# xiezhy6/PASTA-GAN-plusplus

Measured on AMD Instinct MI355X. Metric: 512-res try-on images/sec (SynthesisNetwork fwd), higher is better.
Workload: dtype f32

## Files before the change

### include/pasta_gan_ops.h

```cpp
#ifndef PASTA_GAN_OPS_H
#define PASTA_GAN_OPS_H

#include <stdint.h>

#ifdef __cplusplus
extern "C" {
#endif

#define PG_ABI_VERSION 20

enum pg_dtype { PG_F32 = 0, PG_F16 = 1, PG_BF16 = 2, PG_F64 = 3 };

enum pg_error {
    PG_OK = 0,
    PG_ERR_INVALID_ARG = -1,
    PG_ERR_UNSUPPORTED = -2,
    PG_ERR_TOO_LARGE = -3
};

enum pg_act {
    PG_ACT_LINEAR = 1, PG_ACT_RELU = 2, PG_ACT_LRELU = 3, PG_ACT_TANH = 4, PG_ACT_SIGMOID = 5,
    PG_ACT_ELU = 6, PG_ACT_SELU = 7, PG_ACT_SOFTPLUS = 8, PG_ACT_SWISH = 9
};

int pg_bias_act(const void* x, const void* b, const void* xref, const void* yref, const void* dy, void* y,
                int dtype, int64_t sizeX, int sizeB, int64_t stepB,
                int grad, int act, float alpha, float gain, float clamp, void* stream);
int pg_bias_act_abi_version(void);

int64_t pg_bias_act_grad_bias_workspace(int dtype, int64_t sizeX, int sizeB, int64_t stepB);
int pg_bias_act_grad_bias(const void* dy, const void* yref, void* dx, void* db, void* workspace, int64_t workspace_bytes,
                          int dtype, int64_t sizeX, int sizeB, int64_t stepB,
                          int act, float alpha, float gain, float clamp, void* stream);

int pg_upfirdn2d(const void* x, const float* f, void* y, int dtype,
                 int N, int C, int inH, int inW, const int64_t xstride[4],
                 int fh, int fw, const int64_t fstride[2],
                 int outH, int outW, const int64_t ystride[4],
                 int upx, int upy, int downx, int downy, int padx0, int pady0,
                 int flip, float gain, void* stream);
int pg_upfirdn2d_with_odd_samples(const void* x, const float* f, void* y, float* y_odd, int dtype,
                                  int N, int C, int inH, int inW, const int64_t xstride[4],
// ... 83 lines not shown
    const float* w2[PG_MODCONV_PREP_MAX_JOBS];
    const float* styles[PG_MODCONV_PREP_MAX_JOBS];
    float*       out[PG_MODCONV_PREP_MAX_JOBS];
    float*       s_norm[PG_MODCONV_PREP_MAX_JOBS];
    void*        s16[PG_MODCONV_PREP_MAX_JOBS];
    int          cout[PG_MODCONV_PREP_MAX_JOBS];
    int          cin[PG_MODCONV_PREP_MAX_JOBS];
    int          flags[PG_MODCONV_PREP_MAX_JOBS];
    int          njobs;
    int          half_dtype;
} pg_modconv_prep_jobs;
int pg_modconv_prep_batched(const pg_modconv_prep_jobs* jobs, int N, void* stream);

int pg_conv2d_up2_forward(const float* x, const float* packed, float* y, int N, int Cin, int H, int W, int Cout,
                          const int64_t ystride[4], const float* in_scale, const float* out_scale, void* stream);
int pg_conv2d_up2_splitk_plan(int N, int Cin, int H, int W, int Cout);
int pg_conv2d_up2_forward_splitk(const float* x, const float* packed, float* y, int N, int Cin, int H, int W, int Cout,
                                 const int64_t ystride[4], const float* in_scale, const float* out_scale, float* workspace, int ksplit, void* stream);

int64_t pg_conv2d_up2x3_packed_size(int Cout, int Cin);
int pg_conv2d_up2x3_pack_weight(const float* packed, void* packed_x3, int Cout, int Cin, void* stream);
int pg_conv2d_up2x3_forward(const float* x, const float* packed, const void* packed_x3, float* y, int N, int Cin, int H, int W, int Cout,
                            const int64_t ystride[4], const float* in_scale, const float* out_scale, float* edge_column, void* stream);

int64_t pg_conv2d_stem7x3_packed_size(int Cout);
int pg_conv2d_stem7x3_pack_weight(const float* w, void* packed, int Cout, float scale, int flip_hw, void* stream);
int pg_conv2d_stem7x3_forward(const float* x, const void* packed, float* y, int N, int H, int W, int Cout, const int64_t ystride[4],
                              const pg_conv2d_fusion* fusion, void* stream);

int64_t pg_conv2d_s2x3_packed_size(int Cout, int Cin);
int pg_conv2d_s2x3_pack_weight(const float* packed, void* packed_x3, int Cout, int Cin, void* stream);
int pg_conv2d_s2x3_forward(const float* x, const void* packed_x3, float* y, int N, int Cin, int H, int W, int Cout, const int64_t ystride[4],
                           const pg_conv2d_fusion* fusion, void* stream);

int pg_conv1x1_small(const float* x, const float* w, const float* styles, const float* bias, const float* skip, float* y,
                     int N, int Cin, int64_t HW, int Cout, float scale, float clamp, void* stream);

int pg_conv1x1_fold_prep(const float* wm, const float* bm, const float* wh, const float* bh, const float* styles, float* w_out, float* b_out,
                         int N, int Cm, int C, int Cout, void* stream);
int pg_conv1x1_fold_heads(const float* x, const float* x2, const float* w, const float* bias, const float* skip, float* y_a, float* y_b,
                          int N, int C1, int C2, int64_t HW, int Cout, int c_a, int n_skip, float clamp, void* stream);

int pg_conv3x3_fold_head(const float* xa, const float* xb, const float* w, const float* bias, const float* skip, float* y,
                         int N, int C, int H, int W, int Cout, float clamp, void* stream);

int pg_conv3x3_cin1(const float* x, const float* w, float* y, int N, int H, int W, int Cout, float scale, int act, void* stream);

int pg_instance_norm_stats(const float* x, float* mean, float* rstd, int NC, int64_t HW, float eps, void* stream);
int pg_spade_norm(const float* x, const float* mean, const float* rstd, const float* gamma, const float* beta,
                  float* y, int NC, int64_t HW, void* stream);

#define PG_STATS16_MAX_CHUNKS 256
int pg_instance_norm_stats_cl16(const void* x, float* mean, float* rstd, float* workspace, int dtype, int N, int64_t HW, int C, float eps, void* stream);
int pg_spade_combine_cl16(const void* x, const float* mean, const float* rstd, const void* gamma_beta, void* y, int dtype, int N, int64_t HW, int C,
                          int act, float alpha, float gain, float clamp, void* stream);

int pg_spade_train_forward(const float* x, const float* mean, const float* rstd, const float* gamma, const float* beta, float* y,
                           int N, int C, int64_t HW, int64_t gamma_sample_stride, int64_t beta_sample_stride, void* stream);
int pg_spade_train_backward(const float* dy, const float* x, const float* mean, const float* rstd, const float* gamma, float* sums,
                            float* dx, float* dgamma, float* dbeta, int N, int C, int64_t HW,
                            int64_t gamma_sample_stride, int64_t dgamma_sample_stride, int64_t dbeta_sample_stride, void* stream);

int pg_spade_masked_sums(const float* feat, const float* mask, const float* denorm_mask, float* sums, float* counts,
                         int N, int C, int H, int W, void* stream);
int pg_spade_feat_assemble(const float* feat_upper, const float* feat_lower, const float* mask_upper, const float* mask_lower,
                           const float* denorm_mask_upper, const float* denorm_mask_lower,
// ... 251 lines not shown
```

### pasta-gan-plusplus_amd/torch_utils/custom_ops.py

```python

import concurrent.futures
import ctypes
import fcntl
import glob
import hashlib
import os
import re
import shutil
import subprocess
import sys

verbosity = 'brief'

CSRC_DIR = os.path.normpath(os.path.join(os.path.dirname(os.path.abspath(__file__)), '..', 'csrc'))
INCLUDE_DIR = os.path.normpath(os.path.join(CSRC_DIR, '..', '..', 'include'))
DEV_DIR = os.path.join(CSRC_DIR, 'dev')
OFFLOAD_ARCH = 'gfx950'
HIPCC_FLAGS = ['-O3', '-std=c++17', '-fPIC', '-fvisibility=hidden', f'--offload-arch={OFFLOAD_ARCH}']

PLUGIN_SOURCES = {
    'bias_act_plugin': ['bias_act.hip'],
    'upfirdn2d_plugin': ['upfirdn2d.hip'],
    'patch_routing_plugin': ['patch_routing.hip'],
    'augment_plugin': ['augment.hip'],
    'tryon_plugin': ['tryon.hip'],
    'tryon_front_plugin': ['tryon_front.hip'],
    'train_fetch_plugin': ['train_fetch.hip'],
    'snapshot_grid_plugin': ['snapshot_grid.hip'],
    'vgg_loss_plugin': ['vgg_loss.hip'],
    'image_metrics_plugin': ['image_metrics.hip'],
    'conv2d_plugin': ['conv2d.hip', 'conv2d_inst_k3s1.hip', 'conv2d_inst_k1s1.hip', 'conv2d_inst_k2x2.hip', 'conv2d_inst_k2x1.hip',
                      'conv2d_inst_k1x2.hip', 'conv2d_inst_k7s1.hip', 'conv2d_inst_k3s2.hip', 'conv2d_inst_k1s2.hip', 'conv2d_inst_wino.hip', 'conv2d_inst_wino4.hip', 'conv2d_inst_wino4s.hip', 'conv2d_inst_wino4t.hip', 'conv2d_inst_wino4x.hip', 'conv2d_inst_wino4xs.hip', 'conv2d_inst_wino4xt.hip', 'conv2d_inst_wino4b.hip', 'conv2d_inst_wino4bs.hip', 'conv2d_inst_up2.hip', 'conv2d_inst_stem7.hip', 'conv2d_inst_s2x3.hip', 'conv2d_inst_s1x1.hip',
                      'conv2d_wgrad.hip', 'conv2d16.hip', 'conv2d16_inst_k3s1.hip', 'conv2d16_inst_k3s1b.hip', 'conv2d16_inst_k1s1.hip', 'conv2d16_inst_k2x2.hip', 'conv2d16_inst_k2x1.hip',
                      'conv2d16_inst_k1x2.hip', 'conv2d16_inst_k3s2.hip', 'conv2d16_inst_up2f.hip', 'conv1x1_head16.hip', 'spade16.hip', 'conv1x1_fold.hip', 'conv3x3_fold.hip', 'optim.hip'],
}

ABI_VERSION = 20

_cached_plugins = dict()


class NativePlugin:

    def __init__(self, name, path, abi_name=None):
        self.name = name
        self.path = path
        self.lib = ctypes.CDLL(path)
        probe = getattr(self.lib, 'pg_' + (abi_name or name).replace('_plugin', '') + '_abi_version', None)
        if probe is None:
            raise RuntimeError(f'{path} does not export its ABI version; rebuild it from csrc/')
        probe.restype = ctypes.c_int
        if probe() != ABI_VERSION:
            raise RuntimeError(f'{path} implements ABI version {probe()}, the bindings expect {ABI_VERSION}; rebuild it from csrc/')

    def __repr__(self):
        return f'<NativePlugin {self.name} at {self.path}>'


def _find_hipcc():
    for cand in (os.environ.get('HIPCC'), shutil.which('hipcc'), '/opt/rocm/bin/hipcc'):
        if cand and os.path.isfile(cand):
            return cand
    return None


def _digest(sources, extra_flags):
    h = hashlib.md5()
    deps = sorted(set(list(sources) + glob.glob(os.path.join(CSRC_DIR, '*.h')) + glob.glob(os.path.join(INCLUDE_DIR, '*.h'))))
    for path in deps:
        h.update(os.path.basename(path).encode())
# ... 180 lines not shown
```

### pasta-gan-plusplus_amd/torch_utils/ops/conv2d_gradfix.py

```python

import contextlib
import os

import weakref

import torch

from . import _native as nat
from . import bias_act
from . import conv2d_mfma
from . import conv2d_mfma16

native_input_gradients = os.environ.get('PG_NATIVE_DGRAD', '1') == '1'
native_weight_gradients16 = os.environ.get('PG_NATIVE_WGRAD16', '1') == '1'
native_weight_gradients = os.environ.get('PG_NATIVE_WGRAD', '1') == '1'
enabled = True
weight_gradients_disabled = False


@contextlib.contextmanager
def no_weight_gradients():
    global weight_gradients_disabled
    old = weight_gradients_disabled
    weight_gradients_disabled = True
# ... 117 lines not shown
    if hit is None:
        w = weight.detach()
        if not w.is_contiguous():
            w = w.contiguous()
        hit = conv2d_mfma.pack_weight(w, flip=flip, transpose_oi=transpose_oi, winograd=winograd)
        if sum(e[1].numel() * e[1].element_size() for e in _pack_cache.values()) + hit.numel() * hit.element_size() > _PACK_CACHE_MAX_BYTES:
            _pack_cache.clear()

        def _evict(ref, key=key):
            e = _pack_cache.get(key)
            if e is not None and e[0] is ref:
                del _pack_cache[key]
        _pack_cache[key] = (weakref.ref(base, _evict), hit)
    return hit


def _epilogue_backward(ctx, dy, y, ep, want_b):
    act, alpha, gain, clamp = ep
    if want_b:
        return bias_act._BiasActGrad.apply(dy, None, None, y, 1, act, alpha, gain, clamp, True)
    return bias_act._BiasActGrad.apply(dy, None, None, y, 1, act, alpha, gain, clamp), None


class _Conv2dMfma(torch.autograd.Function):
    @staticmethod
    def forward(ctx, x, weight, bias, stride, padding, transposed, output_padding, ep=None):
        x = x.contiguous()
        n, cin, h, w = x.shape
        kh, kw = int(weight.shape[2]), int(weight.shape[3])
        if not transposed:
            cout = int(weight.shape[0])
            fz = dict(act=ep[0], alpha=ep[1], gain=ep[2], clamp=ep[3] if ep[3] >= 0 else None) if ep is not None else {}
            wg = conv2d_mfma.use_winograd(kh, kw, stride, cout, cin, pad=padding, hw=(h, w), ep=fz)
            y = conv2d_mfma.conv2d_forward(x, _packed(weight, wg), cout, kh, kw, stride=stride, pad=padding, bias=bias, winograd=wg, s2x3=False, **fz)
        else:
            assert ep is None
            cout = int(weight.shape[1])
            out_hw = ((h - 1) * stride - 2 * padding[0] + kh + output_padding[0], (w - 1) * stride - 2 * padding[1] + kw + output_padding[1])
            if ((kh, kw, stride) == (3, 3, 2) and tuple(padding) == (0, 0) and tuple(output_padding) == (0, 0) and bias is None and UP2_TRANSPOSED
                    and (n * cout * out_hw[0] * ((out_hw[1] + 3) // 4 * 4)) * 4 < 2 ** 31):
                main = _packed(weight, 0, flip=False, transpose_oi=True)
                packs = dict(main=main)
                if UP2_TRANSPOSED_X3 and cin % 16 == 0 and cin >= 32:
                    hit = _x3_of_pack.get(id(main))
                    if hit is None or hit[0]() is not main:
                        x3 = conv2d_mfma.pack_s2x3_planes(main, cout, cin)
                        _x3_of_pack[id(main)] = hit = (weakref.ref(main, lambda r, k=id(main): _x3_of_pack.pop(k, None)), x3)
                    packs['x3'] = hit[1]
                y = conv2d_mfma.conv_up2_forward(x, packs, cout, x3=None if 'x3' in packs else False)
            else:
                phases = conv2d_mfma.pack_transposed(weight, stride, padding, (h, w), out_hw)
                y = conv2d_mfma.conv_transpose2d_forward(x, phases, cout, out_hw, stride=stride, bias=bias)
        ctx.save_for_backward(x, weight, y if ep is not None else None)
        ctx.cfg = (stride, padding, transposed, output_padding, bias is not None, ep)
        return y

    @staticmethod
    def backward(ctx, dy):
        x, weight, y = ctx.saved_tensors
        stride, padding, transposed, output_padding, has_bias, ep = ctx.cfg
        kh, kw = int(weight.shape[2]), int(weight.shape[3])
        dx = dw = db = None
        if ep is not None:
            dy, db = _epilogue_backward(ctx, dy, y, ep, has_bias and ctx.needs_input_grad[2])
        if ctx.needs_input_grad[0] and native_input_gradients:
            dx = _input_gradient(dy, x.shape, weight, stride, padding, transposed, output_padding)
        want_w = ctx.needs_input_grad[1] and not weight_gradients_disabled
# ... 92 lines not shown
            if not transposed:
                g = conv2d_mfma16.weight_gradient(x, dy, weight.shape, padding, stride=stride)
            else:
                g = conv2d_mfma16.weight_gradient(dy, x, weight.shape, padding, stride=stride)
            dw = g.to(weight.dtype) if g is not None else None
        if want_b and db is None and (dw is not None or not want_w):
            db = bias_act.channel_sum(dy, 1)
        need_x = dx is None and ctx.needs_input_grad[0]
        need_w = want_w and dw is None
        need_b = want_b and db is None
        if need_x or need_w or need_b:
            gx, gw, gb = torch.ops.aten.convolution_backward(
                dy, x, weight.to(x.dtype), [weight.shape[1 if transposed else 0]] if has_bias else None,
                [stride, stride], list(padding), [1, 1], transposed, list(output_padding), 1, [need_x, need_w, need_b])
            dx = gx if need_x else dx
            dw = gw.to(weight.dtype) if need_w else dw
            db = gb if need_b else db
        return dx, dw, db, None, None, None, None, None


def _input_gradient(dy, x_shape, weight, stride, padding, transposed, output_padding, fn=None, mod=None):
    _Conv2dMfma, conv2d_mfma = (fn or globals()['_Conv2dMfma']), (mod or globals()['conv2d_mfma'])
    kh, kw = int(weight.shape[2]), int(weight.shape[3])
    _, _, h, w = x_shape
    if not transposed:
        if stride == 1:
            py, px = kh - 1 - padding[0], kw - 1 - padding[1]
            if min(py, px) < 0 or not conv2d_mfma.supported(kh, kw, 1):
                return None
            if fn is None and not (torch.is_grad_enabled() and (dy.requires_grad or weight.requires_grad)):
                cin_f = int(weight.shape[1])
                wg = globals()['conv2d_mfma'].use_winograd(kh, kw, 1, cin_f, int(weight.shape[0]), pad=(py, px), hw=dy.shape[2:])
                pk = _packed(weight, wg, flip=True, transpose_oi=True)
                return globals()['conv2d_mfma'].conv2d_forward(dy.contiguous(), pk, cin_f, kh, kw, stride=1, pad=(py, px), winograd=wg)
            return _Conv2dMfma.apply(dy, weight.transpose(0, 1).flip([2, 3]), None, 1, (py, px), False, (0, 0))
        opad = (h - ((dy.shape[2] - 1) * stride - 2 * padding[0] + kh), w - ((dy.shape[3] - 1) * stride - 2 * padding[1] + kw))
        if min(opad) < 0 or max(opad) >= stride or kh < stride or kw < stride:
            return None
        if not all(conv2d_mfma.supported(-(-(kh - a) // stride), -(-(kw - b) // stride), 1) for a in range(stride) for b in range(stride)):
            return None
        return _Conv2dMfma.apply(dy, weight, None, stride, padding, True, opad)
    if not conv2d_mfma.supported(kh, kw, stride) or min(padding) < 0:
        return None
    dx = _Conv2dMfma.apply(dy, weight, None, stride, padding, False, (0, 0))
    return dx if dx.shape[2:] == tuple(x_shape[2:]) else None
```

### pasta-gan-plusplus_amd/torch_utils/ops/conv2d_mfma.py

```python

import contextlib
import ctypes
import os
import weakref

import torch

from .. import custom_ops
from . import _native as nat

ACT_INDEX = {'linear': 1, 'relu': 2, 'lrelu': 3, 'tanh': 4, 'sigmoid': 5, 'elu': 6, 'selu': 7, 'softplus': 8, 'swish': 9}

FUSED_ACTS = ('linear', 'relu', 'lrelu')

SUPPORTED = {(3, 3, 1), (1, 1, 1), (2, 2, 1), (2, 1, 1), (1, 2, 1), (7, 7, 1), (3, 3, 2), (1, 1, 2)}


class Fusion(ctypes.Structure):
    _fields_ = [
        ('in_scale', ctypes.c_void_p), ('in_bias', ctypes.c_void_p), ('in_act', ctypes.c_int), ('in_alpha', ctypes.c_float),
        ('in_gain', ctypes.c_float), ('in_clamp', ctypes.c_float),
        ('out_scale', ctypes.c_void_p), ('noise', ctypes.c_void_p), ('noise_batch_stride', ctypes.c_int64), ('noise_gain', ctypes.c_float),
        ('bias', ctypes.c_void_p), ('act', ctypes.c_int), ('alpha', ctypes.c_float), ('gain', ctypes.c_float), ('clamp', ctypes.c_float),
        ('residual', ctypes.c_void_p),
# ... 90 lines not shown
        lib.pg_conv2d_wgrad_plan.argtypes = [i] * 8
        lib.pg_conv2d_wgrad.restype = i
        lib.pg_conv2d_wgrad.argtypes = [vp, vp, vp, vp] + [i] * 13 + [vp]
        lib.pg_conv2d_up2_forward.restype = i
        lib.pg_conv2d_up2_forward.argtypes = [vp, vp, vp, i, i, i, i, i, ctypes.POINTER(ctypes.c_int64), vp, vp, vp]
        lib.pg_split3_bf16_cl.restype = i
        lib.pg_split3_bf16_cl.argtypes = [vp, vp, i, i, i64, vp]
        lib.pg_conv2d16_wgrad_x3.restype = i
        lib.pg_conv2d16_wgrad_x3.argtypes = [vp, vp, vp, vp] + [i] * 13 + [vp]
        lib.pg_conv2d16_wgrad_plan.restype = i
        lib.pg_conv2d16_wgrad_plan.argtypes = [i] * 8
        lib.pg_conv2d_up2_splitk_plan.restype = i
        lib.pg_conv2d_up2_splitk_plan.argtypes = [i, i, i, i, i]
        lib.pg_conv2d_up2x3_packed_size.restype = i64
        lib.pg_conv2d_up2x3_packed_size.argtypes = [i, i]
        lib.pg_conv2d_up2x3_pack_weight.restype = i
        lib.pg_conv2d_up2x3_pack_weight.argtypes = [vp, vp, i, i, vp]
        lib.pg_conv2d_up2x3_forward.restype = i
        lib.pg_conv2d_up2x3_forward.argtypes = [vp, vp, vp, vp, i, i, i, i, i, ctypes.POINTER(ctypes.c_int64), vp, vp, vp, vp]
        lib.pg_conv2d_up2_forward_splitk.restype = i
        lib.pg_conv2d_up2_forward_splitk.argtypes = [vp, vp, vp, i, i, i, i, i, ctypes.POINTER(ctypes.c_int64), vp, vp, vp, i, vp]
        lib.pg_conv2d_stem7x3_packed_size.restype = i64
        lib.pg_conv2d_stem7x3_packed_size.argtypes = [i]
        lib.pg_conv2d_stem7x3_pack_weight.restype = i
        lib.pg_conv2d_stem7x3_pack_weight.argtypes = [vp, vp, i, ctypes.c_float, i, vp]
        lib.pg_conv2d_stem7x3_forward.restype = i
        lib.pg_conv2d_stem7x3_forward.argtypes = [vp, vp, vp, i, i, i, i, ctypes.POINTER(ctypes.c_int64), ctypes.POINTER(Fusion), vp]
        lib.pg_conv2d_s2x3_packed_size.restype = i64
        lib.pg_conv2d_s2x3_packed_size.argtypes = [i, i]
        lib.pg_conv2d_s2x3_pack_weight.restype = i
        lib.pg_conv2d_s2x3_pack_weight.argtypes = [vp, vp, i, i, vp]
        lib.pg_conv2d_s2x3_forward.restype = i
        lib.pg_conv2d_s2x3_forward.argtypes = [vp, vp, vp, i, i, i, i, i, ctypes.POINTER(i64), ctypes.POINTER(Fusion), vp]
        lib.pg_conv3x3_cin1.restype = i
        lib.pg_conv3x3_cin1.argtypes = [vp, vp, vp, i, i, i, i, f, i, vp]
        lib.pg_conv1x1_small.restype = i
        lib.pg_conv1x1_small.argtypes = [vp] * 6 + [i, i, i64, i, f, f, vp]
        lib.pg_conv1x1_fold_prep.restype = i
        lib.pg_conv1x1_fold_prep.argtypes = [vp] * 7 + [i, i, i, i, vp]
        lib.pg_conv1x1_fold_heads.restype = i
        lib.pg_conv1x1_fold_heads.argtypes = [vp] * 7 + [i, i, i, i64, i, i, i, f, vp]
        lib.pg_conv3x3_fold_head.restype = i
        lib.pg_conv3x3_fold_head.argtypes = [vp] * 6 + [i, i, i, i, i, f, vp]
        _plugin = plugin
    return _plugin


WINO_F2, WINO_F4, WINO_F4B, WINO_F4X3 = 1, 2, 3, 4
WINO_FORMS = {0: ('direct', False, False), WINO_F2: ('winograd', False, False), WINO_F4: ('winograd4', True, False),
              WINO_F4B: ('winograd4', False, True), WINO_F4X3: ('winograd4x3', True, False)}


def _wino_form(winograd):
    if int(winograd) not in WINO_FORMS:
        raise nat.NativeOpError(f'conv2d_mfma: winograd={winograd!r} is not one of the forms {sorted(WINO_FORMS)}')
    return (int(winograd), *WINO_FORMS[int(winograd)])


_WINO4B = os.environ.get('PG_WINO4B', '1')
F4_FORM = WINO_F4 if _WINO4B == '0' else WINO_F4B
F4_WIDE = WINO_F4 if os.environ.get('PG_WINO4_X3', '1') == '0' else WINO_F4X3


def f4_form(hw):
    if _WINO4B == '2':
        return WINO_F4B
# ... 68 lines not shown
        with torch.cuda.device(w.device):
            st = lib.pg_conv2d_winograd_pack_weight(form, nat.ptr(w), nat.ptr(packed), cout, cin, float(scale), int(bool(flip)), int(bool(transpose_oi)), nat.stream_of(w))
        nat.check(st, 'pg_conv2d_winograd_pack_weight')
        return packed
    packed = torch.empty([lib.pg_conv2d_packed_size(cout, cin, kh, kw)], dtype=torch.float32, device=w.device)
    with torch.cuda.device(w.device):
        st = lib.pg_conv2d_pack_weight(nat.ptr(w), nat.ptr(packed), cout, cin, kh, kw, float(scale), int(bool(flip)), int(bool(transpose_oi)), nat.stream_of(w))
    nat.check(st, 'pg_conv2d_pack_weight')
    return packed


S2_X3 = os.environ.get('PG_S2_X3', '1') != '0'
_s2x3_of_pack = {}


def s2x3_wanted(n, cin, cout, h, w):
    if not S2_X3 or os.environ.get('PG_S2_X3', '1') == '0' or cin % 16 != 0 or cin < 32 or h < 3 or w < 3:
        return False
    return True


def pack_s2x3(packed32, cout, cin):
    hit = _s2x3_of_pack.get(id(packed32))
    if hit is not None and hit[0]() is packed32:
        return hit[1]
    lib = _init().lib
    x3 = torch.empty([lib.pg_conv2d_s2x3_packed_size(cout, cin)], dtype=torch.uint8, device=packed32.device)
    with torch.cuda.device(packed32.device):
        nat.check(lib.pg_conv2d_s2x3_pack_weight(nat.ptr(packed32), nat.ptr(x3), cout, cin, nat.stream_of(packed32)), 'pg_conv2d_s2x3_pack_weight')
    _s2x3_of_pack[id(packed32)] = (weakref.ref(packed32, lambda r, k=id(packed32): _s2x3_of_pack.pop(k, None)), x3)
    return x3


def conv2d_forward(x, packed, cout, kh, kw, stride=1, pad=(0, 0), out_hw=None, y=None, out_step=(1, 1), out_off=(0, 0),
                   in_scale=None, in_bias=None, in_act='linear', in_alpha=0.0, in_gain=1.0, in_clamp=None,
                   out_scale=None, noise=None, noise_gain=1.0, bias=None, act='linear', alpha=0.0, gain=1.0, clamp=None,
                   residual=None, spade=None, x2=None, winograd=False, stats_eps=None, s2x3=None):
    lib = _init().lib
    form, label, has_stats_tail, _ = _wino_form(winograd)
    x = _f32c(x, 'x')
    n, cin, h, w = x.shape
    cin_split = 0
    if x2 is not None:
        x2 = _f32c(x2, 'x2')
        if x2.shape[0] != n or x2.shape[2:] != x.shape[2:] or cin % 16 != 0:
            raise nat.NativeOpError('conv2d_mfma: x2 must match x in N, H, W and x must have a multiple of 16 channels')
        cin_split, cin = cin, cin + x2.shape[1]
    pad_y, pad_x = pad
    if out_hw is None:
        out_hw = ((h + 2 * pad_y - kh) // stride + 1, (w + 2 * pad_x - kw) // stride + 1)
    oh, ow = out_hw
    ychan = cout // 2 if spade is not None else cout
    if y is None:
        assert tuple(out_step) == (1, 1) and tuple(out_off) == (0, 0)
        y = torch.empty([n, ychan, oh, ow], dtype=torch.float32, device=x.device)
    else:
        assert y.dtype == torch.float32 and y.device == x.device and y.shape[0] == n and y.shape[1] == ychan
    fz = Fusion()
    keep = []

    def dev(t, name, numel=None):
        t = _f32c(t, name)
        if t is None:
            return None
        if numel is not None and t.numel() != numel:
            raise nat.NativeOpError(f'conv2d_mfma: {name} has {t.numel()} elements, expected {numel}')
        keep.append(t)
        return t.data_ptr()

    fz.in_scale = dev(in_scale, 'in_scale', n * cin)
# ... 18 lines not shown
    if residual is not None:
        if residual.dtype != torch.float32 or residual.shape != y.shape or residual.stride() != y.stride():
            raise nat.NativeOpError('conv2d_mfma: residual must match y in dtype, shape and strides')
        keep.append(residual)
        fz.residual = residual.data_ptr()
    if spade is not None:
        sx, smean, srstd = spade
        if sx.dtype != torch.float32 or sx.shape != y.shape or sx.stride() != y.stride() or smean.numel() != n * ychan or srstd.numel() != n * ychan:
            raise nat.NativeOpError('conv2d_mfma: spade tensors must match the [N, C, OH, OW] output')
        keep += [sx, smean, srstd]
        fz.spade_x, fz.spade_mean, fz.spade_rstd = sx.data_ptr(), smean.data_ptr(), srstd.data_ptr()
    if x2 is not None:
        keep.append(x2)
        fz.x2, fz.cin_split = x2.data_ptr(), cin_split
    stats_part = None
    if stats_eps is not None:
        if not has_stats_tail or spade is not None or in_scale is not None or noise is not None or residual is not None or x2 is not None or in_act != 'linear':
            raise nat.NativeNotCovered('conv2d_mfma: output statistics are gathered by the F(4x4) kernel\'s plain tail only')
        stats_T = lib.pg_conv2d_winograd4_stats_tiles(int(oh), int(ow))
        stats_part = torch.empty([n * cout * stats_T * 2], dtype=torch.float32, device=x.device)
        fz.stats_partial = stats_part.data_ptr()
    with torch.cuda.device(x.device):
        if _timeline is not None:
            ev0, ev1 = torch.cuda.Event(enable_timing=True), torch.cuda.Event(enable_timing=True)
            ev0.record()
        s2x3 = (s2x3 is not False and not form and (kh, kw, int(stride)) == (3, 3, 2) and (int(pad_y), int(pad_x)) == (0, 0) and tuple(out_step) == (1, 1) and tuple(out_off) == (0, 0)
                and (int(oh), int(ow)) == ((h - 3) // 2 + 1, (w - 3) // 2 + 1) and not torch.is_grad_enabled() and residual is None and spade is None and x2 is None
                and in_scale is None and in_bias is None and out_scale is None and noise is None and in_act == 'linear' and float(in_gain) == 1.0 and in_clamp is None
                and act in FUSED_ACTS and s2x3_wanted(n, cin, cout, h, w))
        st = -2
        if s2x3:
            st = lib.pg_conv2d_s2x3_forward(nat.ptr(x), nat.ptr(pack_s2x3(packed, cout, cin)), nat.ptr(y), n, cin, h, w, cout, nat.i64arr(y.stride()), ctypes.byref(fz), nat.stream_of(x))
            s2x3 = st != -2
        if s2x3:
            pass
        elif form:
            if (kh, kw, int(stride)) != (3, 3, 1) or tuple(out_step) != (1, 1) or tuple(out_off) != (0, 0):
                raise nat.NativeOpError('conv2d_mfma: winograd=True needs a 3x3 stride-1 dense-output launch')
            st = lib.pg_conv2d_winograd_forward(form, nat.ptr(x), nat.ptr(packed), nat.ptr(y), n, cin, h, w, cout, int(pad_y), int(pad_x),
                                                int(oh), int(ow), nat.i64arr(y.stride()), ctypes.byref(fz), nat.stream_of(x))
        else:
            ksplit = 1
            if spade is None and x2 is None and os.environ.get('PG_CONV_SPLITK', '1') != '0':
                ksplit = lib.pg_conv2d_splitk_plan(n, cin, int(oh), int(ow), cout, kh, kw, int(stride))
            if ksplit > 1:
                ws = torch.empty([ksplit * n * cout * int(oh) * int(ow)], dtype=torch.float32, device=x.device)
                st = lib.pg_conv2d_forward_splitk(nat.ptr(x), nat.ptr(packed), nat.ptr(y), n, cin, h, w, cout, kh, kw, int(stride), int(pad_y), int(pad_x),
                                                  int(oh), int(ow), nat.i64arr(y.stride()), int(out_step[0]), int(out_step[1]), int(out_off[0]), int(out_off[1]),
                                                  ctypes.byref(fz), nat.ptr(ws), ksplit, nat.stream_of(x))
            else:
                st = lib.pg_conv2d_forward(nat.ptr(x), nat.ptr(packed), nat.ptr(y), n, cin, h, w, cout, kh, kw, int(stride), int(pad_y), int(pad_x),
                                           int(oh), int(ow), nat.i64arr(y.stride()), int(out_step[0]), int(out_step[1]), int(out_off[0]), int(out_off[1]),
                                           ctypes.byref(fz), nat.stream_of(x))
        if _timeline is not None:
            ev1.record()
            _timeline.append(((kh, kw, int(stride), label, f'N{n} {cin}->{cout} {h}x{w}' + (' spade' if spade is not None else '') + (' xf' if in_act != 'linear' else '') + (' mod' if in_scale is not None else '') + (' res' if residual is not None else '') + (' s2x3' if s2x3 else '')), 2.0 * n * cout * oh * ow * cin * kh * kw, ev0, ev1,
                              4 * (x.numel() + (x2.numel() if x2 is not None else 0) + n * ychan * oh * ow)))
    nat.check(st, 'pg_conv2d_forward')
    if stats_part is not None:
        mean = torch.empty([n * cout], dtype=torch.float32, device=x.device)
        rstd = torch.empty_like(mean)
        with torch.cuda.device(x.device):
            st = lib.pg_instance_norm_finish(nat.ptr(stats_part), nat.ptr(mean), nat.ptr(rstd), n * cout, stats_T, int(oh), int(ow), float(stats_eps), nat.stream_of(x))
        nat.check(st, 'pg_instance_norm_finish')
        return y, (mean, rstd)
    return y


def pack_spade_gamma_beta(w_gamma, w_beta, scale_gamma=1.0, scale_beta=1.0, winograd=False):
    c = int(w_gamma.shape[0])
    grp = 32
    assert w_gamma.shape == w_beta.shape and c % 32 == 0
    if _wino_form(winograd)[3]:
        gw, bw = w_gamma.detach() * scale_gamma, w_beta.detach() * scale_beta
        return pack_weight(torch.stack([gw, bw], dim=1).reshape(2 * c, *w_gamma.shape[1:]).contiguous(), winograd=winograd)
    g = (w_gamma.detach() * scale_gamma).reshape(c // grp, grp, *w_gamma.shape[1:])
    b = (w_beta.detach() * scale_beta).reshape(c // grp, grp, *w_beta.shape[1:])
    return pack_weight(torch.cat([g, b], dim=1).reshape(2 * c, *w_gamma.shape[1:]).contiguous(), winograd=winograd)


def transposed_phases(kh, kw, stride, pad_y, pad_x, in_hw, out_hw):
    s = stride

    def axis(k, pad, n_out):
        res = []
        for a in range(s):
            j = -(-(k - a) // s)
            if j <= 0:
                return None
# ... 521 lines not shown
```

Before: 295.4.

## Add bf16x3 split-precision MFMA kernel for 1x1 stride-1 convolutions

```diff
diff --git a/include/pasta_gan_ops.h b/include/pasta_gan_ops.h
--- a/include/pasta_gan_ops.h
+++ b/include/pasta_gan_ops.h
@@ -7,7 +7,7 @@
 extern "C" {
 #endif
 
-#define PG_ABI_VERSION 20
+#define PG_ABI_VERSION 21
 
 enum pg_dtype { PG_F32 = 0, PG_F16 = 1, PG_BF16 = 2, PG_F64 = 3 };
 
@@ -157,6 +157,11 @@
 int pg_conv2d_s2x3_pack_weight(const float* packed, void* packed_x3, int Cout, int Cin, void* stream);
 int pg_conv2d_s2x3_forward(const float* x, const void* packed_x3, float* y, int N, int Cin, int H, int W, int Cout, const int64_t ystride[4],
                            const pg_conv2d_fusion* fusion, void* stream);
+
+int64_t pg_conv1x1_x3_packed_size(int Cout, int Cin);
+int pg_conv1x1_x3_pack_weight(const float* packed, void* packed_x3, int Cout, int Cin, void* stream);
+int pg_conv1x1_x3_forward(const float* x, const float* x2, int cin1, const void* packed_x3, float* y, int N, int Cin, int H, int W, int Cout,
+                          const int64_t ystride[4], const pg_conv2d_fusion* fusion, void* stream);
 
 int pg_conv1x1_small(const float* x, const float* w, const float* styles, const float* bias, const float* skip, float* y,
                      int N, int Cin, int64_t HW, int Cout, float scale, float clamp, void* stream);
diff --git a/pasta-gan-plusplus_amd/csrc/conv1x1_x3.h b/pasta-gan-plusplus_amd/csrc/conv1x1_x3.h
--- /dev/null
+++ b/pasta-gan-plusplus_amd/csrc/conv1x1_x3.h
@@ -0,0 +1,291 @@
+#pragma once
+#include "conv2d_kernel.h"
+
+namespace pgconv {
+
+constexpr int CX_KC = 16;
+constexpr int CX_TP = 128;
+constexpr int CX_NA = CX_TP / 32;
+constexpr int CX_GROUP = 128;
+constexpr int CX_AHEAD = 5;
+constexpr int CX_WREG = CX_AHEAD * 2048;
+constexpr int CX_RAW = 4 * CX_WREG;
+constexpr int CX_PLB = 2 * CX_TP * 16;
+constexpr int CX_MAXCOUT = 1024;
+constexpr int CX_FRAG = 64 * 16;
+constexpr int CX_WSLAB = 3 * CX_FRAG;
+constexpr size_t CX_LDS = (size_t)CX_RAW + 2 * 3 * (size_t)CX_PLB + CX_MAXCOUT * 4;
+
+struct C1x3Params {
+    const float* x; const float* x2; float* y; const unsigned char* wx3; const float* bias;
+    int N, Cin, Cin1, H, W, Cout;
+    int tilesP, groups, total_tiles;
+    int64_t ys[4];
+    int act; float alpha, gain, clamp;
+};
+
+typedef __bf16 cx_bf16x8 __attribute__((ext_vector_type(8)));
+typedef unsigned cx_u32x4 __attribute__((ext_vector_type(4)));
+
+__device__ __forceinline__ void cx_split_pair(float va, float vb, unsigned& p0, unsigned& p1, unsigned& p2) {
+    const unsigned ua = __float_as_uint(va), ub = __float_as_uint(vb);
+    const float ra = va - __uint_as_float(ua & 0xffff0000u), rb = vb - __uint_as_float(ub & 0xffff0000u);
+    const unsigned ura = __float_as_uint(ra), urb = __float_as_uint(rb);
+    const float la = ra - __uint_as_float(ura & 0xffff0000u), lb = rb - __uint_as_float(urb & 0xffff0000u);
+    p0 = __builtin_amdgcn_perm(ub, ua, 0x07060302u);
+    p1 = __builtin_amdgcn_perm(urb, ura, 0x07060302u);
+    p2 = __builtin_amdgcn_perm(__float_as_uint(lb), __float_as_uint(la), 0x07060302u);
+}
+
+__global__ __launch_bounds__(512, 1) void conv1x1_x3(C1x3Params p) {
+    extern __shared__ __attribute__((aligned(16))) unsigned char cx_smem[];
+    float* raw = (float*)cx_smem;
+    unsigned char* planes = cx_smem + CX_RAW;
+    float* bias_s = (float*)(planes + 2 * 3 * CX_PLB);
+
+    const int wave = __builtin_amdgcn_readfirstlane((int)threadIdx.x >> 6);
+    const int lane = (int)threadIdx.x & 63;
+    const unsigned smem_b = __builtin_amdgcn_readfirstlane(lds_offset((const float*)cx_smem));
+    const int HW = p.H * p.W;
+    const int nchunks = p.Cin / CX_KC;
+    const int total = p.total_tiles;
+    const int q8 = total >> 3, r8 = total & 7;
+    const int my_tiles = (total - (int)blockIdx.x + (int)gridDim.x - 1) / (int)gridDim.x;
+    const int my_chunks = my_tiles * nchunks;
+
+    auto decode = [&](int tile, int& n, int& p0, int& grp) __attribute__((always_inline)) {
+        const int xcd = tile & 7;
+        int L = (xcd < r8 ? xcd * (q8 + 1) : r8 * (q8 + 1) + (xcd - r8) * q8) + (tile >> 3);
+        grp = L % p.groups; L /= p.groups;
+        p0 = (L % p.tilesP) * CX_TP;
+        n = L / p.tilesP;
+    };
+
+    for (int c = (int)threadIdx.x; c < p.groups * CX_GROUP; c += 512) bias_s[c] = (p.bias && c < p.Cout) ? p.bias[c] : 0.f;
+    __syncthreads();
+
+    if (wave >= 4) {
+        const int pw = wave - 4;
+        const int kh = pw >> 1, ph = pw & 1;
+        const unsigned reg_b = smem_b + (unsigned)pw * CX_WREG;
+        unsigned xoff[2] = {0x80000000u, 0x80000000u};
+        uint64_t b1 = (uint64_t)(uintptr_t)p.x, b2 = b1;
+        int c_tile = blockIdx.x, c_chunk = 0, c_slot = 0, c_left = my_chunks;
+        auto request = [&]() __attribute__((always_inline)) {
+            if (c_left > 0 && c_chunk == 0) {
+                int n, p0, grp;
+                decode(c_tile, n, p0, grp);
+                b1 = (uint64_t)(uintptr_t)(p.x + (int64_t)n * p.Cin1 * HW);
+                b2 = p.x2 ? (uint64_t)(uintptr_t)(p.x2 + (int64_t)n * (p.Cin - p.Cin1) * HW) : b1;
+                int ll = lane;
+                asm volatile("" : "+v"(ll));
+                const int pix = p0 + 64 * ph + 4 * (ll & 15);
+#pragma unroll
+                for (int i = 0; i < 2; i++)
+                    xoff[i] = pix < HW ? (unsigned)((4 * i + (ll >> 4)) * HW + pix) * 4u : 0x80000000u;
+            }
+            if (c_left <= 0) xoff[0] = xoff[1] = 0x80000000u;
+            const int c0 = c_chunk * CX_KC;
+            const bool second = c0 >= p.Cin1;
+            const uint64_t base = second ? b2 : b1;
+            i32x4 rs;
+            rs[0] = __builtin_amdgcn_readfirstlane((int)(unsigned)base);
+            rs[1] = __builtin_amdgcn_readfirstlane((int)(unsigned)(base >> 32) & 0xffff);
+            rs[2] = __builtin_amdgcn_readfirstlane((second ? p.Cin - p.Cin1 : p.Cin1) * HW * 4);
+            rs[3] = 0x00020000;
+            const int soff = __builtin_amdgcn_readfirstlane(((second ? c0 - p.Cin1 : c0) + 8 * kh) * HW * 4);
+            asm volatile("s_nop 4" : "+s"(rs) :: "memory");
+#pragma unroll
+            for (int i = 0; i < 2; i++) dma_dwordx4_buf(rs, reg_b + (unsigned)c_slot * 2048u + 1024u * i, xoff[i], soff);
+            c_left--;
+            if (++c_slot == CX_AHEAD) c_slot = 0;
+            if (++c_chunk == nchunks) { c_chunk = 0; c_tile += gridDim.x; }
+        };
+        int s_slot = 0;
+        auto split = [&](int g) __attribute__((always_inline)) {
+            const float* rp = raw + (pw * CX_WREG + s_slot * 2048) / 4 + lane;
+            cx_u32x4 pl[3];
+#pragma unroll
+            for (int j = 0; j < 4; j++) {
+                const int ca = 2 * j, cb = ca + 1;
+                const float va = rp[(ca >> 2) * 256 + (ca & 3) * 64], vb = rp[(cb >> 2) * 256 + (cb & 3) * 64];
+                unsigned p0, p1, p2;
+                cx_split_pair(va, vb, p0, p1, p2);
+                pl[0][j] = p0; pl[1][j] = p1; pl[2][j] = p2;
+            }
+            unsigned char* dst = planes + (size_t)(g & 1) * 3 * CX_PLB + (size_t)(kh * CX_TP + 64 * ph + lane) * 16;
+            *(cx_u32x4*)(dst) = pl[0];
+            *(cx_u32x4*)(dst + CX_PLB) = pl[1];
+            *(cx_u32x4*)(dst + 2 * CX_PLB) = pl[2];
+            if (++s_slot == CX_AHEAD) s_slot = 0;
+        };
+#pragma unroll
+        for (int a = 0; a < CX_AHEAD; a++) request();
+        for (int g = 0; g < my_chunks; g++) {
+            asm volatile("s_waitcnt vmcnt(%0)" :: "n"(2 * (CX_AHEAD - 1)) : "memory");
+            split(g);
+            asm volatile("s_waitcnt lgkmcnt(0)" ::: "memory");
+            request();
+            asm volatile("s_barrier" ::: "memory");
+        }
+        asm volatile("s_barrier" ::: "memory");
+        asm volatile("s_waitcnt vmcnt(0)" ::: "memory");
+        return;
+    }
+
+    const int half = lane >> 5, l31 = lane & 31;
+    f32x16 acc[CX_NA], accs[CX_NA];
+    cx_u32x4 A[3];
+    auto wslab = [&](int grp, int chunk) __attribute__((always_inline)) {
+        return p.wx3 + (((int64_t)grp * nchunks + chunk) * 4 + wave) * (int64_t)CX_WSLAB + lane * 16;
+    };
+    int tile = blockIdx.x;
+    int e_n, e_p0, e_grp;
+    decode(tile, e_n, e_p0, e_grp);
+    {
+        const unsigned char* w0 = wslab(e_grp, 0);
+#pragma unroll
+        for (int pl = 0; pl < 3; pl++) A[pl] = *(const cx_u32x4*)(w0 + pl * CX_FRAG);
+        __builtin_amdgcn_s_waitcnt(0x0f70);
+#pragma unroll
+        for (int pl = 0; pl < 3; pl++) asm volatile("" : "+v"(A[pl]));
+    }
+    const float gain = p.gain;
+    const float cl = p.clamp >= 0.f ? p.clamp : __builtin_inff();
+    const float slope = act_slope(p.act, p.alpha);
+    const int cs_ = (int)p.ys[1], rs_ = (int)p.ys[2], xs_ = (int)p.ys[3];
+    asm volatile("s_barrier" ::: "memory");
+    for (int ti = 0, g = 0; ti < my_tiles; ti++) {
+#pragma unroll
+        for (int a = 0; a < CX_NA; a++)
+#pragma unroll
+            for (int k = 0; k < 16; k++) acc[a][k] = accs[a][k] = 0.f;
+        int nx_n = e_n, nx_p0 = e_p0, nx_grp = e_grp;
+        if (ti + 1 < my_tiles) decode(tile + (int)gridDim.x, nx_n, nx_p0, nx_grp);
+        for (int k = 0; k < nchunks; k++, g++) {
+            const unsigned char* wn = k + 1 < nchunks ? wslab(e_grp, k + 1) : wslab(nx_grp, 0);
+            const unsigned char* bb = planes + (size_t)(g & 1) * 3 * CX_PLB + (size_t)(half * CX_TP + l31) * 16;
+            cx_u32x4 B[CX_NA][3];
+#pragma unroll
+            for (int pl = 0; pl < 3; pl++)
+#pragma unroll
+                for (int a = 0; a < CX_NA; a++) B[a][pl] = *(const cx_u32x4*)(bb + (size_t)pl * CX_PLB + (size_t)a * 32 * 16);
+            constexpr int PA[6] = {2, 1, 1, 0, 0, 0}, PB[6] = {0, 1, 0, 2, 1, 0};
+            f32x16 accp[CX_NA];
+#pragma unroll
+            for (int pr = 0; pr < 6; pr++) {
+#pragma unroll
+                for (int a = 0; a < CX_NA; a++) {
+                    if (pr < 5) {
+                        accs[a] = __builtin_amdgcn_mfma_f32_32x32x16_bf16(__builtin_bit_cast(cx_bf16x8, A[PA[pr]]), __builtin_bit_cast(cx_bf16x8, B[a][PB[pr]]), accs[a], 0, 0, 0);
+                    } else {
+                        f32x16 z;
+#pragma unroll
+                        for (int q = 0; q < 16; q++) z[q] = 0.f;
+                        accp[a] = __builtin_amdgcn_mfma_f32_32x32x16_bf16(__builtin_bit_cast(cx_bf16x8, A[0]), __builtin_bit_cast(cx_bf16x8, B[a][0]), z, 0, 0, 0);
+                    }
+                }
+                if (pr == 0 || pr == 2 || pr == 5) {
+                    __builtin_amdgcn_sched_barrier(0);
+                    A[PA[pr]] = *(const cx_u32x4*)(wn + PA[pr] * CX_FRAG);
+                    __builtin_amdgcn_sched_barrier(0);
+                }
+            }
+#pragma unroll
+            for (int a = 0; a < CX_NA; a++)
+#pragma unroll
+                for (int q = 0; q < 16; q++) acc[a][q] += accp[a][q];
+            asm volatile("s_waitcnt lgkmcnt(0)\n\ts_barrier" ::: "memory");
+        }
+
+        {
+            __builtin_amdgcn_s_waitcnt(0x0f70);
+#pragma unroll
+            for (int pl = 0; pl < 3; pl++) asm volatile("" : "+v"(A[pl]));
+            int ll;
+            asm volatile("v_mbcnt_lo_u32_b32 %0, -1, 0\n\tv_mbcnt_hi_u32_b32 %0, -1, %0" : "=v"(ll));
+            const int half = ll >> 5, l31 = ll & 31;
+            const int co0 = e_grp * CX_GROUP + 32 * wave + 4 * half;
+            i32x4 yrsrc;
+            {
+                const uint64_t base = (uint64_t)(uintptr_t)(p.y + (int64_t)e_n * p.ys[0]);
+                yrsrc[0] = __builtin_amdgcn_readfirstlane((int)(unsigned)base);
+                yrsrc[1] = __builtin_amdgcn_readfirstlane((int)(unsigned)(base >> 32) & 0xffff);
+                yrsrc[2] = 0x7ffffffc;
+                yrsrc[3] = 0x00020000;
+            }
+            asm volatile("s_nop 4" : "+s"(yrsrc) :: "memory");
+            const float* bs = bias_s + co0;
+#pragma unroll
+            for (int a = 0; a < CX_NA; a++) {
+                const int pix = e_p0 + 32 * a + l31;
+                const bool ok = pix < HW;
+                const int oy = pix / p.W, ox = pix - oy * p.W;
+                const unsigned o0 = (unsigned)(co0 * cs_ + oy * rs_ + ox * xs_) * 4u;
+#pragma unroll
+                for (int kq = 0; kq < 4; kq++) {
+                    const f32x4 b4 = *(const f32x4*)(bs + 8 * kq);
+#pragma unroll
+                    for (int j = 0; j < 4; j++) {
+                        float v = (acc[a][4 * kq + j] + accs[a][4 * kq + j]) + b4[j];
+                        v = v > 0.f ? v : v * slope;
+                        v = fminf(fmaxf(v * gain, -cl), cl);
+                        const unsigned off = (ok && co0 + 8 * kq + j < p.Cout) ? o0 + (unsigned)((8 * kq + j) * cs_) * 4u : 0x80000000u;
+                        asm volatile("buffer_store_dword %0, %1, %2, 0 offen" :: "v"(v), "v"(off), "s"(yrsrc) : "memory");
+                    }
+                }
+            }
+        }
+        tile += gridDim.x;
+        e_n = nx_n; e_p0 = nx_p0; e_grp = nx_grp;
+    }
+    asm volatile("s_waitcnt vmcnt(0)" ::: "memory");
+}
+
+__global__ __launch_bounds__(256) void c1x3_pack_kernel(const float* __restrict__ wp32, unsigned short* __restrict__ out, int Cin, int CoutP128, int CoutP32) {
+    const int nchunks = Cin / CX_KC;
+    const int64_t total = (int64_t)Cin * CoutP128;
+    for (int64_t i = (int64_t)blockIdx.x * 256 + threadIdx.x; i < total; i += (int64_t)gridDim.x * 256) {
+        const int co = (int)(i % CoutP128), ci = (int)(i / CoutP128);
+        const float v = co < CoutP32 ? wp32[(int64_t)ci * CoutP32 + co] : 0.f;
+        const unsigned u0 = __float_as_uint(v) & 0xffff0000u;
+        const float r = v - __uint_as_float(u0);
+        const unsigned u1 = __float_as_uint(r) & 0xffff0000u;
+        const unsigned u2 = __float_as_uint(r - __uint_as_float(u1)) & 0xffff0000u;
+        const int grp = co >> 7, mb = (co >> 5) & 3, m = co & 31, chunk = ci >> 4, kh = (ci >> 3) & 1, j = ci & 7;
+        const int64_t dst = (((((int64_t)grp * nchunks + chunk) * 4 + mb) * 3) * 2 + kh) * 256 + m * 8 + j;
+        out[dst] = (unsigned short)(u0 >> 16);
+        out[dst + 512] = (unsigned short)(u1 >> 16);
+        out[dst + 1024] = (unsigned short)(u2 >> 16);
+    }
+}
+
+inline int64_t c1x3_packed_bytes(int Cout, int Cin) { return (int64_t)((Cout + CX_GROUP - 1) / CX_GROUP) * (Cin / CX_KC) * 4 * CX_WSLAB; }
+
+inline bool c1x3_serves(const C1x3Params& p) {
+    const int64_t HW = (int64_t)p.H * p.W;
+    if (p.Cin % CX_KC != 0 || p.Cin < 2 * CX_KC || HW % 4 != 0 || p.Cout > CX_MAXCOUT) return false;
+    if ((((uintptr_t)p.x) | ((uintptr_t)p.x2)) & 15) return false;
+    if (p.x2 ? (p.Cin1 <= 0 || p.Cin1 >= p.Cin || p.Cin1 % CX_KC != 0) : p.Cin1 != p.Cin) return false;
+    return (int64_t)p.Cin * HW * 4 < 0x7fffffffLL;
+}
+
+inline int launch_c1x3(C1x3Params p, hipStream_t s) {
+    if (!c1x3_serves(p) || !p.wx3) return PG_ERR_UNSUPPORTED;
+    const int64_t HW = (int64_t)p.H * p.W;
+    p.tilesP = (int)((HW + CX_TP - 1) / CX_TP);
+    p.groups = (p.Cout + CX_GROUP - 1) / CX_GROUP;
+    const int64_t tiles = (int64_t)p.N * p.tilesP * p.groups;
+    if (tiles > 0x7fffffffLL) return PG_ERR_TOO_LARGE;
+    if (p.ys[1] < 0 || p.ys[2] < 0 || p.ys[3] < 0) return PG_ERR_UNSUPPORTED;
+    if (((int64_t)(p.groups * CX_GROUP) * p.ys[1] + (int64_t)p.H * p.ys[2] + (int64_t)p.W * p.ys[3]) * 4 >= 0x7fffffffLL) return PG_ERR_UNSUPPORTED;
+    p.total_tiles = (int)tiles;
+    const int64_t blocks = tiles < (int64_t)num_cu() ? tiles : (int64_t)num_cu();
+    static PerDeviceOnce once;
+    const hipError_t e = once.run([] { return hipFuncSetAttribute((const void*)conv1x1_x3, hipFuncAttributeMaxDynamicSharedMemorySize, 160 * 1024); });
+    if (e != hipSuccess) return (int)e;
+    hipLaunchKernelGGL(conv1x1_x3, dim3((unsigned)blocks), dim3(512), CX_LDS, s, p);
+    return launch_status();
+}
+
+}
diff --git a/pasta-gan-plusplus_amd/csrc/conv2d_inst_c1x3.hip b/pasta-gan-plusplus_amd/csrc/conv2d_inst_c1x3.hip
--- /dev/null
+++ b/pasta-gan-plusplus_amd/csrc/conv2d_inst_c1x3.hip
@@ -0,0 +1,40 @@
+#include "conv1x1_x3.h"
+
+PG_EXPORT int64_t pg_conv1x1_x3_packed_size(int Cout, int Cin) {
+    if (Cout <= 0 || Cin <= 0 || Cin % 16 != 0) return 0;
+    return pgconv::c1x3_packed_bytes(Cout, Cin);
+}
+
+PG_EXPORT int pg_conv1x1_x3_pack_weight(const float* packed, void* packed_x3, int Cout, int Cin, void* stream) {
+    if (!packed || !packed_x3 || Cout <= 0 || Cin <= 0 || (((uintptr_t)packed_x3) & 15) != 0) return PG_ERR_INVALID_ARG;
+    if (Cin % 16 != 0) return PG_ERR_UNSUPPORTED;
+    const int CoutP32 = (Cout + 31) / 32 * 32, CoutP128 = (Cout + 127) / 128 * 128;
+    const int64_t total = (int64_t)Cin * CoutP128;
+    int64_t blocks = (total + 255) / 256;
+    if (blocks > (int64_t)pg::max_stream_blocks()) blocks = pg::max_stream_blocks();
+    hipLaunchKernelGGL(pgconv::c1x3_pack_kernel, dim3((unsigned)blocks), dim3(256), 0, (hipStream_t)stream, packed, (unsigned short*)packed_x3, Cin, CoutP128, CoutP32);
+    return pg::launch_status();
+}
+
+PG_EXPORT int pg_conv1x1_x3_forward(const float* x, const float* x2, int cin1, const void* packed_x3, float* y, int N, int Cin, int H, int W, int Cout,
+                                    const int64_t ystride[4], const pg_conv2d_fusion* fusion, void* stream) {
+    if (!x || !packed_x3 || !y || !ystride || N <= 0 || Cin <= 0 || H <= 0 || W <= 0 || Cout <= 0 || cin1 <= 0 || cin1 > Cin) return PG_ERR_INVALID_ARG;
+    if ((((uintptr_t)x) & 3) != 0 || (((uintptr_t)x2) & 3) != 0 || (((uintptr_t)y) & 3) != 0 || (((uintptr_t)packed_x3) & 15) != 0) return PG_ERR_INVALID_ARG;
+    if (x2 ? cin1 == Cin : cin1 != Cin) return PG_ERR_INVALID_ARG;
+    pgconv::C1x3Params p;
+    p.x = x; p.x2 = x2; p.y = y; p.wx3 = (const unsigned char*)packed_x3; p.bias = nullptr;
+    p.N = N; p.Cin = Cin; p.Cin1 = cin1; p.H = H; p.W = W; p.Cout = Cout;
+    for (int i = 0; i < 4; i++) p.ys[i] = ystride[i];
+    p.act = PG_ACT_LINEAR; p.alpha = 0.f; p.gain = 1.f; p.clamp = -1.f;
+    if (fusion) {
+        const pg_conv2d_fusion& f = *fusion;
+        if (f.x2 && (f.x2 != x2 || f.cin_split != cin1)) return PG_ERR_INVALID_ARG;
+        if (f.in_scale || f.in_bias || (f.in_act != 0 && f.in_act != PG_ACT_LINEAR) || f.in_clamp >= 0.f || (f.in_gain != 0.f && f.in_gain != 1.f) || f.out_scale || f.noise || f.residual ||
+            f.spade_x || f.spade_mean || f.spade_rstd || f.stats_partial)
+            return PG_ERR_UNSUPPORTED;
+        const int act = f.act == 0 ? PG_ACT_LINEAR : f.act;
+        if (act != PG_ACT_LINEAR && act != PG_ACT_RELU && act != PG_ACT_LRELU) return PG_ERR_UNSUPPORTED;
+        p.bias = f.bias; p.act = act; p.alpha = f.alpha; p.gain = f.gain == 0.f ? 1.f : f.gain; p.clamp = f.clamp;
+    }
+    return pgconv::launch_c1x3(p, (hipStream_t)stream);
+}
diff --git a/pasta-gan-plusplus_amd/torch_utils/custom_ops.py b/pasta-gan-plusplus_amd/torch_utils/custom_ops.py
--- a/pasta-gan-plusplus_amd/torch_utils/custom_ops.py
+++ b/pasta-gan-plusplus_amd/torch_utils/custom_ops.py
@@ -30,12 +30,12 @@
     'vgg_loss_plugin': ['vgg_loss.hip'],
     'image_metrics_plugin': ['image_metrics.hip'],
     'conv2d_plugin': ['conv2d.hip', 'conv2d_inst_k3s1.hip', 'conv2d_inst_k1s1.hip', 'conv2d_inst_k2x2.hip', 'conv2d_inst_k2x1.hip',
-                      'conv2d_inst_k1x2.hip', 'conv2d_inst_k7s1.hip', 'conv2d_inst_k3s2.hip', 'conv2d_inst_k1s2.hip', 'conv2d_inst_wino.hip', 'conv2d_inst_wino4.hip', 'conv2d_inst_wino4s.hip', 'conv2d_inst_wino4t.hip', 'conv2d_inst_wino4x.hip', 'conv2d_inst_wino4xs.hip', 'conv2d_inst_wino4xt.hip', 'conv2d_inst_wino4b.hip', 'conv2d_inst_wino4bs.hip', 'conv2d_inst_up2.hip', 'conv2d_inst_stem7.hip', 'conv2d_inst_s2x3.hip', 'conv2d_inst_s1x1.hip',
+                      'conv2d_inst_k1x2.hip', 'conv2d_inst_k7s1.hip', 'conv2d_inst_k3s2.hip', 'conv2d_inst_k1s2.hip', 'conv2d_inst_wino.hip', 'conv2d_inst_wino4.hip', 'conv2d_inst_wino4s.hip', 'conv2d_inst_wino4t.hip', 'conv2d_inst_wino4x.hip', 'conv2d_inst_wino4xs.hip', 'conv2d_inst_wino4xt.hip', 'conv2d_inst_wino4b.hip', 'conv2d_inst_wino4bs.hip', 'conv2d_inst_up2.hip', 'conv2d_inst_stem7.hip', 'conv2d_inst_s2x3.hip', 'conv2d_inst_c1x3.hip', 'conv2d_inst_s1x1.hip',
                       'conv2d_wgrad.hip', 'conv2d16.hip', 'conv2d16_inst_k3s1.hip', 'conv2d16_inst_k3s1b.hip', 'conv2d16_inst_k1s1.hip', 'conv2d16_inst_k2x2.hip', 'conv2d16_inst_k2x1.hip',
                       'conv2d16_inst_k1x2.hip', 'conv2d16_inst_k3s2.hip', 'conv2d16_inst_up2f.hip', 'conv1x1_head16.hip', 'spade16.hip', 'conv1x1_fold.hip', 'conv3x3_fold.hip', 'optim.hip'],
 }
 
-ABI_VERSION = 20
+ABI_VERSION = 21
 
 _cached_plugins = dict()
 
diff --git a/pasta-gan-plusplus_amd/torch_utils/ops/conv2d_gradfix.py b/pasta-gan-plusplus_amd/torch_utils/ops/conv2d_gradfix.py
--- a/pasta-gan-plusplus_amd/torch_utils/ops/conv2d_gradfix.py
+++ b/pasta-gan-plusplus_amd/torch_utils/ops/conv2d_gradfix.py
@@ -173,7 +173,7 @@
             cout = int(weight.shape[0])
             fz = dict(act=ep[0], alpha=ep[1], gain=ep[2], clamp=ep[3] if ep[3] >= 0 else None) if ep is not None else {}
             wg = conv2d_mfma.use_winograd(kh, kw, stride, cout, cin, pad=padding, hw=(h, w), ep=fz)
-            y = conv2d_mfma.conv2d_forward(x, _packed(weight, wg), cout, kh, kw, stride=stride, pad=padding, bias=bias, winograd=wg, s2x3=False, **fz)
+            y = conv2d_mfma.conv2d_forward(x, _packed(weight, wg), cout, kh, kw, stride=stride, pad=padding, bias=bias, winograd=wg, s2x3=False, c1x3=False, **fz)
         else:
             assert ep is None
             cout = int(weight.shape[1])
@@ -332,7 +332,7 @@
                 cin_f = int(weight.shape[1])
                 wg = globals()['conv2d_mfma'].use_winograd(kh, kw, 1, cin_f, int(weight.shape[0]), pad=(py, px), hw=dy.shape[2:])
                 pk = _packed(weight, wg, flip=True, transpose_oi=True)
-                return globals()['conv2d_mfma'].conv2d_forward(dy.contiguous(), pk, cin_f, kh, kw, stride=1, pad=(py, px), winograd=wg)
+                return globals()['conv2d_mfma'].conv2d_forward(dy.contiguous(), pk, cin_f, kh, kw, stride=1, pad=(py, px), winograd=wg, c1x3=False)
             return _Conv2dMfma.apply(dy, weight.transpose(0, 1).flip([2, 3]), None, 1, (py, px), False, (0, 0))
         opad = (h - ((dy.shape[2] - 1) * stride - 2 * padding[0] + kh), w - ((dy.shape[3] - 1) * stride - 2 * padding[1] + kw))
         if min(opad) < 0 or max(opad) >= stride or kh < stride or kw < stride:
diff --git a/pasta-gan-plusplus_amd/torch_utils/ops/conv2d_mfma.py b/pasta-gan-plusplus_amd/torch_utils/ops/conv2d_mfma.py
--- a/pasta-gan-plusplus_amd/torch_utils/ops/conv2d_mfma.py
+++ b/pasta-gan-plusplus_amd/torch_utils/ops/conv2d_mfma.py
@@ -146,6 +146,12 @@
         lib.pg_conv2d_s2x3_pack_weight.argtypes = [vp, vp, i, i, vp]
         lib.pg_conv2d_s2x3_forward.restype = i
         lib.pg_conv2d_s2x3_forward.argtypes = [vp, vp, vp, i, i, i, i, i, ctypes.POINTER(i64), ctypes.POINTER(Fusion), vp]
+        lib.pg_conv1x1_x3_packed_size.restype = i64
+        lib.pg_conv1x1_x3_packed_size.argtypes = [i, i]
+        lib.pg_conv1x1_x3_pack_weight.restype = i
+        lib.pg_conv1x1_x3_pack_weight.argtypes = [vp, vp, i, i, vp]
+        lib.pg_conv1x1_x3_forward.restype = i
+        lib.pg_conv1x1_x3_forward.argtypes = [vp, vp, i, vp, vp, i, i, i, i, i, ctypes.POINTER(i64), ctypes.POINTER(Fusion), vp]
         lib.pg_conv3x3_cin1.restype = i
         lib.pg_conv3x3_cin1.argtypes = [vp, vp, vp, i, i, i, i, f, i, vp]
         lib.pg_conv1x1_small.restype = i
@@ -280,10 +286,35 @@
     return x3
 
 
+C1_X3 = os.environ.get('PG_C1_X3', '1') != '0'
+_c1x3_of_pack = {}
+_C1X3_NOT_FASTER = frozenset({(64, 128, 256 * 256)})
+
+
+def c1x3_wanted(n, cin, cout, h, w):
+    if not C1_X3 or os.environ.get('PG_C1_X3', '1') == '0' or cin % 16 != 0 or cin < 32 or (h * w) % 4 != 0 or cout > 1024:
+        return False
+    if h * w >= 512 * 512 or (cin, cout, h * w) in _C1X3_NOT_FASTER:
+        return False
+    return True
+
+
+def pack_c1x3(packed32, cout, cin):
+    hit = _c1x3_of_pack.get(id(packed32))
+    if hit is not None and hit[0]() is packed32:
+        return hit[1]
+    lib = _init().lib
+    x3 = torch.empty([lib.pg_conv1x1_x3_packed_size(cout, cin)], dtype=torch.uint8, device=packed32.device)
+    with torch.cuda.device(packed32.device):
+        nat.check(lib.pg_conv1x1_x3_pack_weight(nat.ptr(packed32), nat.ptr(x3), cout, cin, nat.stream_of(packed32)), 'pg_conv1x1_x3_pack_weight')
+    _c1x3_of_pack[id(packed32)] = (weakref.ref(packed32, lambda r, k=id(packed32): _c1x3_of_pack.pop(k, None)), x3)
+    return x3
+
+
 def conv2d_forward(x, packed, cout, kh, kw, stride=1, pad=(0, 0), out_hw=None, y=None, out_step=(1, 1), out_off=(0, 0),
                    in_scale=None, in_bias=None, in_act='linear', in_alpha=0.0, in_gain=1.0, in_clamp=None,
                    out_scale=None, noise=None, noise_gain=1.0, bias=None, act='linear', alpha=0.0, gain=1.0, clamp=None,
-                   residual=None, spade=None, x2=None, winograd=False, stats_eps=None, s2x3=None):
+                   residual=None, spade=None, x2=None, winograd=False, stats_eps=None, s2x3=None, c1x3=None):
     lib = _init().lib
     form, label, has_stats_tail, _ = _wino_form(winograd)
     x = _f32c(x, 'x')
@@ -368,7 +399,15 @@
         if s2x3:
             st = lib.pg_conv2d_s2x3_forward(nat.ptr(x), nat.ptr(pack_s2x3(packed, cout, cin)), nat.ptr(y), n, cin, h, w, cout, nat.i64arr(y.stride()), ctypes.byref(fz), nat.stream_of(x))
             s2x3 = st != -2
-        if s2x3:
+        c1x3 = (c1x3 is not False and not s2x3 and not form and (kh, kw, int(stride)) == (1, 1, 1) and (int(pad_y), int(pad_x)) == (0, 0) and tuple(out_step) == (1, 1)
+                and tuple(out_off) == (0, 0) and (int(oh), int(ow)) == (h, w) and not torch.is_grad_enabled() and residual is None and spade is None
+                and in_scale is None and in_bias is None and out_scale is None and noise is None and in_act == 'linear' and float(in_gain) == 1.0 and in_clamp is None
+                and stats_eps is None and act in FUSED_ACTS and (x2 is None or cin_split % 16 == 0) and c1x3_wanted(n, cin, cout, h, w))
+        if c1x3:
+            st = lib.pg_conv1x1_x3_forward(nat.ptr(x), nat.ptr(x2) if x2 is not None else None, cin_split if x2 is not None else cin, nat.ptr(pack_c1x3(packed, cout, cin)),
+                                           nat.ptr(y), n, cin, h, w, cout, nat.i64arr(y.stride()), ctypes.byref(fz), nat.stream_of(x))
+            c1x3 = st != -2
+        if s2x3 or c1x3:
             pass
         elif form:
             if (kh, kw, int(stride)) != (3, 3, 1) or tuple(out_step) != (1, 1) or tuple(out_off) != (0, 0):
@@ -390,7 +429,7 @@
                                            ctypes.byref(fz), nat.stream_of(x))
         if _timeline is not None:
             ev1.record()
-            _timeline.append(((kh, kw, int(stride), label, f'N{n} {cin}->{cout} {h}x{w}' + (' spade' if spade is not None else '') + (' xf' if in_act != 'linear' else '') + (' mod' if in_scale is not None else '') + (' res' if residual is not None else '') + (' s2x3' if s2x3 else '')), 2.0 * n * cout * oh * ow * cin * kh * kw, ev0, ev1,
+            _timeline.append(((kh, kw, int(stride), label, f'N{n} {cin}->{cout} {h}x{w}' + (' spade' if spade is not None else '') + (' xf' if in_act != 'linear' else '') + (' mod' if in_scale is not None else '') + (' res' if residual is not None else '') + (' s2x3' if s2x3 else '') + (' c1x3' if c1x3 else '')), 2.0 * n * cout * oh * ow * cin * kh * kw, ev0, ev1,
                               4 * (x.numel() + (x2.numel() if x2 is not None else 0) + n * ychan * oh * ow)))
     nat.check(st, 'pg_conv2d_forward')
     if stats_part is not None:
```

Measured after the change: 297.6, median of 6. About the same (+0.7%).
